# DixianZhu/deBWT

Hardware: NVIDIA B200
Metric: bwt_build_throughput (higher is better)
Workload: dtype u64

## Files before the change

### debwt_b200/csrc/api.cu

```cuda
#include <algorithm>
#include <cstring>
#include <map>
#include <mutex>
#include <string>
#include <tuple>
#include <vector>

#include "../../include/debwt_b200.h"
#include "../../include/debwt_b200_dev.h"
#include "radix_sort.cuh"
#include "stages.cuh"
#include "special.cuh"
#include "ctx.cuh"
#include "dist_kernels.cuh"

namespace debwt {

static thread_local std::string g_err;
unsigned g_launches = 0;
unsigned long long g_launches_total = 0;
void set_error(const std::string& msg) { g_err = msg; }

#define FAIL(msg)            \
    do {                     \
// ... 293 lines not shown
    }
    mark();

    u64 *d_ka = nullptr, *d_kb = nullptr;
    if (dalloc(pool, &d_ka, nk + 2) || dalloc(pool, &d_kb, nk + 2)) return -1;
    if (k_extract(d_text, n, d_seps, R, d_ka, st)) return -1;
    mark();

    void* d_sortws = nullptr;
    if (pool.alloc(&d_sortws, sort_workspace_bytes(nk, c->sort_cfg))) return -1;
    SortWorkspace ws;
    sort_workspace_bind(ws, d_sortws, nk, c->sort_cfg);
    int sweeps = 0;
    ws.ev_sweep_begin = c->ev[11]; ws.ev_sweep_end = c->ev[12]; ws.sweeps_out = &sweeps;
    const unsigned launches_before_sort = g_launches;
    u64* d_keys = nullptr;
    KeyIndex ki;
    ki.bits = key_index_bits(nk);
    if (dalloc(pool, &ki.idx, (1ull << ki.bits) + 2) || k_key_index_init(ki, st)) return -1;
    bool index_marked = false;
    ws.key_index = ki.idx; ws.key_index_bits = ki.bits; ws.key_index_done = &index_marked;
    const bool text_hist = text_digit_hist_applies(n, R);
    if (text_hist && (radix_sort_clear(ws, st) || k_text_digit_hist(d_text, n, d_seps, R, ws.hist, st))) return -1;
    if (radix_sort_u64(d_ka, d_kb, nk, ws, st, &d_keys, text_hist)) return -1;
    S.sort_launches = g_launches - launches_before_sort;
    S.sort_sweeps = (u32)sweeps;
    pool.adopt(d_keys == d_ka ? d_kb : d_ka, (nk + 2) * 8);
    pool.adopt(d_sortws, sort_workspace_bytes(nk, c->sort_cfg));
    u32 h_err[2] = {0, 0};
    CUDA_TRY(cudaMemcpyAsync(h_err, d_err, 8, cudaMemcpyDeviceToHost, st));
    mark();

    u16* d_gmask = nullptr;
    if (dalloc(pool, &d_gmask, nk + 2)) return -1;
    CUDA_TRY(cudaMemsetAsync(d_gmask, 0, (nk + 2) * 2, st));
    if (k_key_index_finish(d_keys, nk, ki, index_marked, st)) return -1;
    if (k_mark_edges(d_keys, nk, ki, d_gmask, st)) return -1;
    if (k_mark_heads_tails(d_text, d_seps, R, d_keys, nk, ki, d_gmask, st)) return -1;
    void* d_brws = nullptr; u64* d_tot = nullptr;
    if (pool.alloc(&d_brws, branch_workspace_bytes(nk)) || dalloc(pool, &d_tot, 4)) return -1;
    if (k_branch_count(d_keys, nk, d_gmask, true, d_brws, d_tot, st)) return -1;
    u64 h_tot[2] = {0, 0};
    CUDA_TRY(cudaMemcpyAsync(h_tot, d_tot, 16, cudaMemcpyDeviceToHost, st));
    CUDA_TRY(cudaStreamSynchronize(st));
    if (h_err[0]) FAIL(c->resolve_ambiguous ? "input contains a symbol that is neither a base nor an IUPAC ambiguity code"
                                            : "input contains a symbol other than A, C, G, T (either case)");
    if (h_err[1] != R) FAIL("input contains '#' or '$' inside a record (they are reserved for the record separators)");
    BranchTable bt;
    bt.n_branch = h_tot[0]; bt.n_blue = h_tot[1];
    S.n_branch = bt.n_branch; S.n_blue = bt.n_blue;
    {
        int bits = 8;
        while (bits < 27 && (1ull << bits) < 2 * bt.n_branch) ++bits;
        bt.bits = bits;
    }
    if (dalloc(pool, &bt.kmer, bt.n_branch + 1) || dalloc(pool, &bt.head, bt.n_branch + 1) ||
        dalloc(pool, &bt.blue, bt.n_branch + 2) || dalloc(pool, &bt.cursor, bt.n_branch + 1) ||
        dalloc(pool, &bt.bidx, BranchTable::index_words(bt.bits)))
        return -1;
    CUDA_TRY(cudaMemsetAsync(bt.cursor, 0, (bt.n_branch + 1) * 4, st));
    if (k_branch_write(d_keys, nk, d_gmask, d_brws, bt, st)) return -1;
    {
        const u32 m32 = (u32)bt.n_blue;
        CUDA_TRY(cudaMemcpyAsync(bt.blue + bt.n_branch, &m32, 4, cudaMemcpyHostToDevice, st));
    }
    if (k_branch_index(bt, st)) return -1;
    int id_bits = 1;
    while (id_bits < 64 && (bt.n_branch >> id_bits)) ++id_bits;
    const bool group_by_sort = id_bits <= 28 && n < (1ull << 32) && bt.n_blue > 1 &&
                               c->blue_grouping == 2;
    bt.hbits = BranchTable::hash_bits(bt.n_branch);
    bt.hmode = group_by_sort ? 0 : 1;
    if (dalloc(pool, &bt.hslots, 1ull << bt.hbits) || k_branch_hash(bt, st)) return -1;
    mark();
// ... 409 lines not shown
    CUDA_TRY(cudaStreamSynchronize(s.st));
    float ms = 0;
    CUDA_TRY(cudaEventElapsedTime(&ms, e0, e1));
    if (ms_out) *ms_out = ms;
    cudaEventDestroy(e0); cudaEventDestroy(e1);
    return 0;
}

int debwt_k_rle(int device, const uint64_t* sorted, uint64_t n, uint64_t* kmers_out, uint64_t* counts_out,
                uint64_t* n_distinct_out) {
    Scratch s;
    if (open_scratch(s, device)) return -1;
    u64 *d_k, *d_km, *d_ct, *d_tot; void* d_ws;
    if (s.get(&d_k, n + 2) || s.get(&d_km, n + 2) || s.get(&d_ct, n + 2) || s.get(&d_tot, 2)) return -1;
    CUDA_TRY(cudaMalloc(&d_ws, rle_workspace_bytes(n)));
    s.ptrs.push_back(d_ws);
    CUDA_TRY(cudaMemcpyAsync(d_k, sorted, n * 8, cudaMemcpyHostToDevice, s.st));
    if (k_rle(d_k, n, d_km, d_ct, d_ws, d_tot, s.st)) return -1;
    u64 d = 0;
    CUDA_TRY(cudaMemcpyAsync(&d, d_tot, 8, cudaMemcpyDeviceToHost, s.st));
    CUDA_TRY(cudaStreamSynchronize(s.st));
    CUDA_TRY(cudaMemcpyAsync(kmers_out, d_km, d * 8, cudaMemcpyDeviceToHost, s.st));
    CUDA_TRY(cudaMemcpyAsync(counts_out, d_ct, d * 8, cudaMemcpyDeviceToHost, s.st));
    CUDA_TRY(cudaStreamSynchronize(s.st));
    if (n_distinct_out) *n_distinct_out = d;
    return 0;
}

int debwt_k_group_masks(int device, const char* text, uint64_t n, const uint64_t* seps, uint64_t R, uint16_t* masks_out) {
    if (check_seps(seps, R, n)) return -1;
    Scratch s;
    if (open_scratch(s, device)) return -1;
    const u64 nk = n - 32 * R;
    u8* d_a; u64 *d_w, *d_s, *d_ka, *d_kb; u32* d_e; u16* d_g; void* d_ws;
    KeyIndex ki;
    ki.bits = key_index_bits(nk);
    if (s.get(&d_a, n + 64) || s.get(&d_w, text_words(n)) || s.get(&d_e, 4) || s.get(&d_s, R) || s.get(&d_ka, nk + 2) ||
        s.get(&d_kb, nk + 2) || s.get(&d_g, nk + 2) || s.get(&ki.idx, (1ull << ki.bits) + 2))
        return -1;
    CUDA_TRY(cudaMalloc(&d_ws, sort_workspace_bytes(nk, 0)));
    s.ptrs.push_back(d_ws);
    SortWorkspace ws;
    sort_workspace_bind(ws, d_ws, nk, 0);
    CUDA_TRY(cudaMemcpyAsync(d_a, text, n, cudaMemcpyHostToDevice, s.st));
    CUDA_TRY(cudaMemcpyAsync(d_s, seps, R * 8, cudaMemcpyHostToDevice, s.st));
    CUDA_TRY(cudaMemsetAsync(d_e, 0, 16, s.st));
    CUDA_TRY(cudaMemsetAsync(d_g, 0, (nk + 2) * 2, s.st));
    u64* d_keys = nullptr;
    if (k_pack(d_a, n, d_w, d_e, s.st) || k_extract(d_w, n, d_s, R, d_ka, s.st) ||
        radix_sort_u64(d_ka, d_kb, nk, ws, s.st, &d_keys) || k_build_key_index(d_keys, nk, ki, s.st) ||
        k_mark_edges(d_keys, nk, ki, d_g, s.st) || k_mark_heads_tails(d_w, d_s, R, d_keys, nk, ki, d_g, s.st) ||
        k_propagate(d_keys, nk, d_g, s.st))
        return -1;
    CUDA_TRY(cudaMemcpyAsync(masks_out, d_g, nk * 2, cudaMemcpyDeviceToHost, s.st));
    CUDA_TRY(cudaStreamSynchronize(s.st));
    return 0;
}


int debwt_k_codes(int device, const char* text, uint64_t n, const uint64_t* seps, uint64_t R, uint8_t* codes_out, uint64_t codes_cap,
                  uint64_t* n_codes_out, uint64_t* blue_head_out, uint64_t* blue_spindex_out, uint8_t* blue_prev_out, uint64_t blue_cap,
                  uint64_t* n_blue_out) {
    debwt_ctx* c = nullptr;
    if (debwt_create(&c, device)) return -1;
    c->cap.on = true;
    int rc = debwt_set_text(c, text, n, seps, R);
    if (!rc) rc = debwt_build(c, 32);
    if (!rc) {
        const auto& q = c->cap;
        if (n_codes_out) *n_codes_out = q.n_codes;
        if (n_blue_out) *n_blue_out = q.blue.size();
        if (q.n_codes > codes_cap || q.blue.size() > blue_cap) { set_error("debwt_k_codes: output buffers too small"); rc = -1; }
    }
    if (!rc) {
        const auto& q = c->cap;
        for (u64 i = 0; i < q.n_codes; ++i) {
            u8 code = (u8)((q.codes[i >> 5] >> (2 * (31 - (i & 31)))) & 3ull);
            if ((q.sep[i >> 5] >> (i & 31)) & 1u) code = i == q.dollar_index ? 5 : 4;
            codes_out[i] = code;
        }
        for (u64 b = 0; b < q.seg_kmer.size(); ++b)
            for (u32 e = q.seg_off[b]; e < q.seg_off[b + 1]; ++e) {
                blue_head_out[e] = q.seg_head[b];
                blue_spindex_out[e] = q.blue[e] >> 4;
                blue_prev_out[e] = (u8)(q.blue[e] & 15ull);
// ... 105 lines not shown
```

### debwt_b200/csrc/stages.cu

```cuda
#include "stages.cuh"

#include <cstdlib>
#include "special.cuh"
#include "stages_dev.cuh"
#include "dist_kernels.cuh"

namespace debwt {

namespace {

constexpr int TPB = 256;
inline unsigned grid_for(u64 work, int per_block) { return (unsigned)((work + per_block - 1) / per_block); }

constexpr int SCAN_ITEMS = 16;
constexpr int SCAN_TILE = TPB * SCAN_ITEMS;

template <bool POPC>
__device__ __forceinline__ u32 scan_f(u32 v) { return POPC ? (u32)__popc(v) : v; }

template <bool POPC>
__global__ void __launch_bounds__(TPB) scan_reduce_kernel(const u32* __restrict__ in, u64 m, u32* __restrict__ part) {
    __shared__ u32 sm[40];
    const u64 base = (u64)blockIdx.x * SCAN_TILE;
    u32 s = 0;
// ... 348 lines not shown
    void* scan_ws = p;
    p += (scan_workspace_bytes(nt) + 7) & ~(size_t)7;
    u64* starts = reinterpret_cast<u64*>(p);
    rle_count_kernel<<<(unsigned)nt, TPB, 0, st>>>(sorted, n, tile_cnt);
    if (scan_exclusive_u32(tile_cnt, tile_ex, nt, false, scan_ws, d_total, st)) return -1;
    rle_write_kernel<<<(unsigned)nt, TPB, 0, st>>>(sorted, n, tile_ex, kmers, starts);
    u64 d = 0;
    CUDA_TRY(cudaMemcpyAsync(&d, d_total, 8, cudaMemcpyDeviceToHost, st));
    CUDA_TRY(cudaStreamSynchronize(st));
    diff_kernel<<<grid_for(d, TPB), TPB, 0, st>>>(starts, d, n, counts);
    DEBWT_COUNT(3);
    CUDA_TRY(cudaGetLastError());
    return 0;
}

namespace {

__global__ void __launch_bounds__(TPB) key_index_mark_kernel(const u64* __restrict__ k, u64 n, KeyIndex ki) {
    const u64 i = (u64)blockIdx.x * TPB + threadIdx.x;
    if (i >= n) return;
    const int sh = 64 - ki.bits;
    const u64 cur = k[i] >> sh;
    if (i == 0 || (k[i - 1] >> sh) != cur) ki.idx[cur] = (u32)i;
}

__global__ void __launch_bounds__(TPB) key_index_fill_kernel(const u64* __restrict__ k, u64 n, KeyIndex ki) {
    const u64 t = (u64)blockIdx.x * TPB + threadIdx.x;
    const u64 nb = 1ull << ki.bits;
    if (t > nb) return;
    if (t == nb) { ki.idx[t] = (u32)n; return; }
    if (ki.idx[t] == 0xFFFFFFFFu) ki.idx[t] = (u32)lower_bound_u64(k, 0, n, t << (64 - ki.bits));
}

constexpr int ME_ROWS = 4;

__device__ __forceinline__ void edge_rows(const u64* __restrict__ k, u64 n, const KeyIndex& ki, u16* __restrict__ gmask, u64 base,
                                          u64 limit) {
    u64 key[ME_ROWS], lo[ME_ROWS], hi[ME_ROWS];
    bool act[ME_ROWS];
#pragma unroll
    for (int j = 0; j < ME_ROWS; ++j) {
        const u64 i = base + (u64)j * TPB;
        act[j] = i < limit;
        key[j] = act[j] ? k[i] : 0;
        if (act[j] && i > 0 && k[i - 1] == key[j]) act[j] = false;
    }
#pragma unroll
    for (int j = 0; j < ME_ROWS; ++j) {
        const u64 t = (key[j] << 2) >> (64 - ki.bits);
        lo[j] = act[j] ? ki.idx[t] : 0;
        hi[j] = act[j] ? ki.idx[t + 1] : 0;
    }
#pragma unroll
    for (int j = 0; j < ME_ROWS; ++j) {
        if (!act[j]) continue;
        const u64 q = key[j] << 2;
        const u64 hs = lower_bound_u64(k, lo[j], hi[j], q);
        if (hs < n && (k[hs] >> 2) == (q >> 2)) atomic_or_u16(gmask, hs, 1u << (u32)(key[j] >> 62));
    }
#pragma unroll
    for (int j = 0; j < ME_ROWS; ++j) {
        if (!act[j]) continue;
        const u64 i = base + (u64)j * TPB;
        atomic_or_u16(gmask, group_head(k, i), 1u << (GM_OUT_SHIFT + (u32)(key[j] & 3)));
    }
}

constexpr u64 ME_TILE = 8192;
constexpr u64 ME_CAP = 8 * ME_TILE;
struct EdgeRun { u64 begin, end; };

__global__ void __launch_bounds__(TPB) edge_bounds_kernel(const u64* __restrict__ k, u64 n, KeyIndex ki, u64 tiles,
                                                         u64* __restrict__ bounds) {
    const u64 x = (u64)blockIdx.x * TPB + threadIdx.x;
    if (x >= 4 * (tiles + 1)) return;
    const u32 c = (u32)(x / (tiles + 1));
    const u64 t = x % (tiles + 1);
    const u64 cbeg = ki.idx[(u64)c << (ki.bits - 2)];
    const u64 cend = (c == 3) ? n : (u64)ki.idx[(u64)(c + 1) << (ki.bits - 2)];
    const u64 a = t * ME_TILE;
    u64 r;
    if (a == 0) r = cbeg;
    else if (a >= n) r = cend;
    else {
        const u64 low = (k[a - 1] >> 2) + 1;
        r = (low >> 62) ? cend : indexed_lower_bound(k, ki, ((u64)c << 62) | low);
    }
    bounds[x] = r;
}

__global__ void __launch_bounds__(TPB) mark_edges_kernel(const u64* __restrict__ k, u64 n, KeyIndex ki, u16* __restrict__ gmask,
                                                        const u64* __restrict__ bounds, u64 tiles, EdgeRun* __restrict__ over,
                                                        u32* __restrict__ n_over) {
    const u32 c = blockIdx.x & 3u;
    const u64 tile = blockIdx.x >> 2;
    const u64 sb = bounds[c * (tiles + 1) + tile];
    u64 se = bounds[c * (tiles + 1) + tile + 1];
    if (se - sb > ME_CAP && se > sb) {
        if (threadIdx.x == 0) over[atomicAdd(n_over, 1u)] = EdgeRun{sb + ME_CAP, se};
        se = sb + ME_CAP;
    }
    for (u64 i0 = sb; i0 < se; i0 += (u64)TPB * ME_ROWS) edge_rows(k, n, ki, gmask, i0 + threadIdx.x, se);
}

__global__ void __launch_bounds__(TPB) mark_edges_over_kernel(const u64* __restrict__ k, u64 n, KeyIndex ki, u16* __restrict__ gmask,
                                                             const EdgeRun* __restrict__ over, const u32* __restrict__ n_over) {
    const u32 m = *n_over;
    for (u32 q = 0; q < m; ++q) {
        const EdgeRun r = over[q];
        for (u64 i0 = r.begin + (u64)blockIdx.x * (TPB * ME_ROWS); i0 < r.end; i0 += (u64)gridDim.x * (TPB * ME_ROWS))
            edge_rows(k, n, ki, gmask, i0 + threadIdx.x, r.end);
    }
}

__global__ void __launch_bounds__(TPB) mark_heads_tails_kernel(const u64* __restrict__ words, const u64* __restrict__ seps,
                                                              u64 n_rec, const u64* __restrict__ k, u64 n, KeyIndex ki,
                                                              u16* __restrict__ gmask) {
    const u64 r = (u64)blockIdx.x * TPB + threadIdx.x;
    if (r >= n_rec) return;
    const u64 start = r ? seps[r - 1] + 1 : 0;
    u64 x = text_window32(words, start) & ~3ull;
    u64 h = indexed_lower_bound(k, ki, x);
    if (h < n && (k[h] & ~3ull) == x) atomic_or_u16(gmask, h, GM_IN_SEP);
    x = text_window32(words, seps[r] - KNODE) & ~3ull;
    h = indexed_lower_bound(k, ki, x);
    if (h < n && (k[h] & ~3ull) == x) atomic_or_u16(gmask, h, GM_OUT_TAIL);
}

__global__ void __launch_bounds__(TPB) propagate_kernel(const u64* __restrict__ k, u64 n, u16* __restrict__ gmask) {
    const u64 i = (u64)blockIdx.x * TPB + threadIdx.x;
    if (i >= n || i == 0) return;
    if ((k[i - 1] >> 2) != (k[i] >> 2)) return;
    gmask[i] = gmask[group_head(k, i)];
}

constexpr int BR_ITEMS = 8;
constexpr int BR_TILE = TPB * BR_ITEMS;

template <bool WRITE, bool PROPAGATE>
__global__ void __launch_bounds__(TPB) branch_kernel(const u64* __restrict__ k, u64 n, u16* __restrict__ gmask,
                                                    u32* __restrict__ tile_nb, u32* __restrict__ tile_blue,
                                                    const u32* __restrict__ tile_nb_ex, const u32* __restrict__ tile_blue_ex,
                                                    u32* __restrict__ head_bits, BranchTable bt) {
    constexpr int NW = TPB / 32;
    __shared__ u32 s_cnt[BR_ITEMS * NW + 1], s_blue[BR_ITEMS * NW + 1];
    if (WRITE && tile_nb[blockIdx.x] == 0) return;
    const int lane = threadIdx.x & 31, warp = threadIdx.x >> 5;
    const u64 base = (u64)blockIdx.x * BR_TILE;
    const u32 lt = lanemask_lt();
    u32 flags[BR_ITEMS], size[BR_ITEMS], bal[BR_ITEMS];
#pragma unroll
    for (int j = 0; j < BR_ITEMS; ++j) {
        const u64 i = base + (u64)j * TPB + threadIdx.x;
        flags[j] = 0;
        size[j] = 0;
        if (WRITE) {
            bal[j] = head_bits[(base + (u64)j * TPB) / 32 + warp];
            if ((bal[j] >> lane) & 1u) {
                const u32 m = gmask[i];
// ... 47 lines not shown
            if (lane >= o) { ic += tc; ib += tb; }
        }
        const u32 ec = ic - (c0 + c1), eb = ib - (b0 + b1);
        s_cnt[2 * lane] = ec; s_cnt[2 * lane + 1] = ec + c0;
        s_blue[2 * lane] = eb; s_blue[2 * lane + 1] = eb + b0;
        if (lane == 31) {
            s_cnt[BR_ITEMS * NW] = ic; s_blue[BR_ITEMS * NW] = ib;
            if (!WRITE) { tile_nb[blockIdx.x] = ic; tile_blue[blockIdx.x] = ib; }
        }
    }
    if (!WRITE) return;
    __syncthreads();
    const u64 ob0 = tile_nb_ex[blockIdx.x];
    const u32 ol0 = tile_blue_ex[blockIdx.x];
#pragma unroll
    for (int j = 0; j < BR_ITEMS; ++j) {
        if (bal[j] == 0) continue;
        u32 inc = size[j];
#pragma unroll
        for (int o = 1; o < 32; o <<= 1) {
            const u32 t = __shfl_up_sync(0xffffffffu, inc, o);
            if (lane >= o) inc += t;
        }
        if (flags[j]) {
            const u64 i = base + (u64)j * TPB + threadIdx.x;
            const u64 ob = ob0 + s_cnt[j * NW + warp] + __popc(bal[j] & lt);
            bt.kmer[ob] = (k[i] & ~3ull) | (flags[j] & 3u);
            bt.head[ob] = (u32)i;
            bt.blue[ob] = ol0 + s_blue[j * NW + warp] + (inc - size[j]);
        }
    }
}

__global__ void __launch_bounds__(TPB) branch_index_kernel(BranchTable bt) {
    const u64 t = (u64)blockIdx.x * TPB + threadIdx.x;
    const u64 nb = 1ull << bt.bits;
    if (t > nb) return;
    bt.bidx[t] = (t == nb) ? (u32)bt.n_branch : (u32)lower_bound_u64(bt.kmer, 0, bt.n_branch, t << (64 - bt.bits));
}

__global__ void __launch_bounds__(TPB) branch_filter_kernel(BranchTable bt) {
    const u64 b = (u64)blockIdx.x * TPB + threadIdx.x;
    if (b >= bt.n_branch) return;
    const u64 f = bt.filter_of(bt.kmer[b] & ~3ull);
    atomicOr(bt.filter() + (f >> 5), 1u << (f & 31));
}

__global__ void __launch_bounds__(TPB) branch_hash_kernel(BranchTable bt) {
    const u64 b = (u64)blockIdx.x * TPB + threadIdx.x;
    if (b >= bt.n_branch) return;
    const u64 e = bt.kmer[b];
    const u64 mask = (1ull << bt.hbits) - 1;
    for (u64 h = bt.hash_of(e & ~3ull);; h = (h + 1) & mask) {
        unsigned long long* claim = reinterpret_cast<unsigned long long*>(&bt.hslots[h].x);
        if (atomicCAS(claim, 0ull, (unsigned long long)e) == 0ull) {
            bt.hslots[h].y = bt.hmode ? (u64)bt.blue[b] << 32 : b;
            return;
        }
    }
}

__global__ void __launch_bounds__(TPB) special_ins_kernel(const u64* __restrict__ k, u64 n, KeyIndex ki,
                                                         const u64* __restrict__ pads, u64 m, u64* __restrict__ ins) {
    const u64 t = (u64)blockIdx.x * TPB + threadIdx.x;
    if (t < m) ins[t] = indexed_upper_bound(k, ki, pads[t]);
}

}

int k_key_index_init(KeyIndex ki, cudaStream_t st) {
    CUDA_TRY(cudaMemsetAsync(ki.idx, 0xFF, ((1ull << ki.bits) + 1) * 4, st));
    return 0;
}

int k_key_index_finish(const u64* sorted, u64 n, KeyIndex ki, bool marked, cudaStream_t st) {
    if (n && !marked) {
        key_index_mark_kernel<<<grid_for(n, TPB), TPB, 0, st>>>(sorted, n, ki);
        DEBWT_COUNT(1);
    }
    key_index_fill_kernel<<<grid_for((1ull << ki.bits) + 1, TPB), TPB, 0, st>>>(sorted, n, ki);
    DEBWT_COUNT(1);
    CUDA_TRY(cudaGetLastError());
    return 0;
}

int k_build_key_index(const u64* sorted, u64 n, KeyIndex ki, cudaStream_t st) {
    if (k_key_index_init(ki, st)) return -1;
    return k_key_index_finish(sorted, n, ki, false, st);
}

int k_mark_edges(const u64* sorted, u64 n, KeyIndex ki, u16* gmask, cudaStream_t st) {
    if (n == 0) return 0;
    const u64 tiles = (n + ME_TILE - 1) / ME_TILE;
    const u64 cap = n / ME_CAP + 8;
    char* ws = nullptr;
    CUDA_TRY(cudaMallocAsync(reinterpret_cast<void**>(&ws), 16 + cap * sizeof(EdgeRun) + 4 * (tiles + 1) * 8, st));
    u32* n_over = reinterpret_cast<u32*>(ws);
    EdgeRun* over = reinterpret_cast<EdgeRun*>(ws + 16);
    u64* bounds = reinterpret_cast<u64*>(ws + 16 + cap * sizeof(EdgeRun));
    cudaMemsetAsync(n_over, 0, 16, st);
    edge_bounds_kernel<<<grid_for(4 * (tiles + 1), TPB), TPB, 0, st>>>(sorted, n, ki, tiles, bounds);
    mark_edges_kernel<<<(unsigned)(4 * tiles), TPB, 0, st>>>(sorted, n, ki, gmask, bounds, tiles, over, n_over);
    mark_edges_over_kernel<<<148 * 8, TPB, 0, st>>>(sorted, n, ki, gmask, over, n_over);
    DEBWT_COUNT(3);
    const cudaError_t e = cudaGetLastError();
    cudaFreeAsync(ws, st);
    if (e != cudaSuccess) { set_error(std::string("mark_edges: ") + cudaGetErrorString(e)); return -1; }
    return 0;
}

int k_mark_heads_tails(const u64* words, const u64* d_seps, u64 n_rec, const u64* sorted, u64 n, KeyIndex ki, u16* gmask,
                       cudaStream_t st) {
    mark_heads_tails_kernel<<<grid_for(n_rec, TPB), TPB, 0, st>>>(words, d_seps, n_rec, sorted, n, ki, gmask);
    DEBWT_COUNT(1);
    CUDA_TRY(cudaGetLastError());
    return 0;
}

int k_propagate(const u64* sorted, u64 n, u16* gmask, cudaStream_t st) {
    if (n == 0) return 0;
    propagate_kernel<<<grid_for(n, TPB), TPB, 0, st>>>(sorted, n, gmask);
    DEBWT_COUNT(1);
    CUDA_TRY(cudaGetLastError());
    return 0;
}

namespace {
struct BranchWs { u32 *nb, *blue, *nb_ex, *blue_ex, *head_bits; void* scan_ws; u64 nt; };
BranchWs branch_ws(void* workspace, u64 n) {
    BranchWs w;
    w.nt = (n + BR_TILE - 1) / BR_TILE;
    u32* p = reinterpret_cast<u32*>(workspace);
    w.nb = p; w.blue = p + w.nt; w.nb_ex = p + 2 * w.nt; w.blue_ex = p + 3 * w.nt;
    char* q = reinterpret_cast<char*>(p + 4 * w.nt);
    q += (8 - (reinterpret_cast<uintptr_t>(q) & 7)) & 7;
    w.scan_ws = q;
    q += (scan_workspace_bytes(w.nt + 1) + 15) & ~(size_t)15;
    w.head_bits = reinterpret_cast<u32*>(q);
    return w;
}
}

size_t branch_workspace_bytes(u64 n) {
    const u64 nt = (n + BR_TILE - 1) / BR_TILE + 1;
    return nt * 16 + 16 + scan_workspace_bytes(nt) + 32 + nt * (BR_TILE / 8);
}

int k_branch_count(const u64* sorted, u64 n, u16* gmask, bool propagate, void* workspace, u64* d_totals, cudaStream_t st) {
    BranchWs w = branch_ws(workspace, n);
    BranchTable none;
    if (propagate) branch_kernel<false, true><<<(unsigned)w.nt, TPB, 0, st>>>(sorted, n, gmask, w.nb, w.blue, nullptr, nullptr, w.head_bits, none);
    else branch_kernel<false, false><<<(unsigned)w.nt, TPB, 0, st>>>(sorted, n, gmask, w.nb, w.blue, nullptr, nullptr, w.head_bits, none);
    DEBWT_COUNT(1);
    if (scan_exclusive_u32(w.nb, w.nb_ex, w.nt, false, w.scan_ws, d_totals, st)) return -1;
    if (scan_exclusive_u32(w.blue, w.blue_ex, w.nt, false, w.scan_ws, d_totals + 1, st)) return -1;
    CUDA_TRY(cudaGetLastError());
    return 0;
}

int k_branch_write(const u64* sorted, u64 n, const u16* gmask, void* workspace, BranchTable bt, cudaStream_t st) {
    BranchWs w = branch_ws(workspace, n);
    branch_kernel<true, false><<<(unsigned)w.nt, TPB, 0, st>>>(sorted, n, const_cast<u16*>(gmask), w.nb, nullptr, w.nb_ex, w.blue_ex, w.head_bits, bt);
    DEBWT_COUNT(1);
    CUDA_TRY(cudaGetLastError());
    return 0;
}

int k_branch_index(BranchTable bt, cudaStream_t st) {
    branch_index_kernel<<<grid_for((1ull << bt.bits) + 1, TPB), TPB, 0, st>>>(bt);
    CUDA_TRY(cudaMemsetAsync(bt.filter(), 0, (1ull << (BranchTable::filter_bits(bt.bits) - 5)) * 4, st));
    if (bt.n_branch) branch_filter_kernel<<<grid_for(bt.n_branch, TPB), TPB, 0, st>>>(bt);
    DEBWT_COUNT(2);
    CUDA_TRY(cudaGetLastError());
    return 0;
}

int k_branch_hash(BranchTable bt, cudaStream_t st) {
    if (!bt.hslots) return 0;
    CUDA_TRY(cudaMemsetAsync(bt.hslots, 0, (1ull << bt.hbits) * sizeof(ulonglong2), st));
    if (bt.n_branch) branch_hash_kernel<<<grid_for(bt.n_branch, TPB), TPB, 0, st>>>(bt);
    DEBWT_COUNT(1);
    CUDA_TRY(cudaGetLastError());
    return 0;
}

namespace {
__global__ void __launch_bounds__(128) special_scan_kernel(const u64* __restrict__ words, const u64* __restrict__ seps,
                                                          u64 n_rec, const u64* __restrict__ k, u64 n_keys, KeyIndex ki,
                                                          SpecialInfo* __restrict__ out) {
// ... 628 lines not shown
```

### debwt_b200/csrc/stages.cuh

```cuda
#pragma once
#include "common.cuh"

namespace debwt {

size_t scan_workspace_bytes(u64 m);
int scan_exclusive_u32(const u32* in, u32* out, u64 m, bool popc, void* workspace, u64* d_total, cudaStream_t st);

struct PackPolicy {
    bool resolve = false;
    u64 seed = 0;
    u64 pos_base = 0;
};
int k_pack(const u8* ascii, u64 n, u64* words, u32* d_err, cudaStream_t st, PackPolicy pol = PackPolicy());
inline u64 text_words(u64 n) { return (n + 32 + 31) / 32 + 1; }
int k_extract(const u64* words, u64 n, const u64* d_seps, u64 n_rec, u64* keys, cudaStream_t st);
int k_extract_slice(const u64* words, u64 n, u64 pos_lo, u64 pos_hi, const u64* d_seps, u64 n_rec, u64 idx_base, u64* keys,
                    cudaStream_t st);

bool text_digit_hist_applies(u64 n, u64 n_rec);
int k_text_digit_hist(const u64* words, u64 n, const u64* d_seps, u64 n_rec, u64* ghist, cudaStream_t st);

int k_rle(const u64* sorted, u64 n, u64* kmers, u64* counts, void* workspace, u64* d_total, cudaStream_t st);
size_t rle_workspace_bytes(u64 n);

struct KeyIndex {
    u32* idx = nullptr;
    int bits = 0;
};
inline int key_index_bits(u64 n) {
    int b = 8;
    while (b < 28 && (8ull << b) < n) ++b;
    return b;
}
int k_build_key_index(const u64* sorted, u64 n, KeyIndex ki, cudaStream_t st);
int k_key_index_init(KeyIndex ki, cudaStream_t st);
int k_key_index_finish(const u64* sorted, u64 n, KeyIndex ki, bool marked, cudaStream_t st);
__host__ __device__ __forceinline__ u64 indexed_lower_bound(const u64* __restrict__ k, const KeyIndex& ki, u64 q) {
    const u64 t = q >> (64 - ki.bits);
    return lower_bound_u64(k, ki.idx[t], ki.idx[t + 1], q);
}
__host__ __device__ __forceinline__ u64 indexed_upper_bound(const u64* __restrict__ k, const KeyIndex& ki, u64 q) {
    const u64 t = q >> (64 - ki.bits);
    return upper_bound_u64(k, ki.idx[t], ki.idx[t + 1], q);
}

int k_mark_edges(const u64* sorted, u64 n, KeyIndex ki, u16* gmask, cudaStream_t st);
int k_mark_heads_tails(const u64* words, const u64* d_seps, u64 n_rec, const u64* sorted, u64 n, KeyIndex ki, u16* gmask,
                       cudaStream_t st);
int k_propagate(const u64* sorted, u64 n, u16* gmask, cudaStream_t st);

struct BranchTable {
    u64 n_branch = 0;
    u64 n_blue = 0;
    u64* kmer = nullptr;
    u32* head = nullptr;
    u32* blue = nullptr;
    u32* cursor = nullptr;
    u32* bidx = nullptr;
    int bits = 0;
    ulonglong2* hslots = nullptr;
    int hbits = 0;
    int hmode = 0;
    __host__ __device__ static int hash_bits(u64 n_branch) { int b = 10; while (b < 40 && (1ull << b) < 3 * n_branch) ++b; return b; }
    __host__ __device__ u64 hash_of(u64 x) const { return ((x >> 2) * 0x9E3779B97F4A7C15ull) >> (64 - hbits); }
    __host__ __device__ u64 filter_of(u64 x) const { return ((x >> 2) * 0x9E3779B97F4A7C15ull) >> (64 - filter_bits(bits)); }
    __host__ __device__ static int filter_bits(int bits) { return bits + 3 < 30 ? bits + 3 : 30; }
    __host__ __device__ static u64 index_words(int bits) { return (1ull << bits) + 2 + (1ull << (filter_bits(bits) - 5)); }
    __host__ __device__ u32* filter() const { return bidx + (1ull << bits) + 2; }
};
size_t branch_workspace_bytes(u64 n);
int k_branch_count(const u64* sorted, u64 n, u16* gmask, bool propagate, void* workspace, u64* d_totals, cudaStream_t st);
int k_branch_write(const u64* sorted, u64 n, const u16* gmask, void* workspace, BranchTable bt, cudaStream_t st);
int k_branch_index(BranchTable bt, cudaStream_t st);
int k_branch_hash(BranchTable bt, cudaStream_t st);

int k_special_insertion(const u64* sorted, u64 n, KeyIndex ki, const u64* pads, u64 m, u64* ins, cudaStream_t st);

int k_flag_positions(const u64* words, u64 n, const u64* d_seps, u64 n_rec, BranchTable bt, u32* mo_bits, u64* blue,
                     cudaStream_t st);
int k_flag_positions_keys(const u64* words, u64 n, const u64* d_seps, u64 n_rec, BranchTable bt, int shift, u32* mo_bits,
                          u64* bkeys, u64* d_counter, cudaStream_t st);
int k_blue_keys_fix(u64* bkeys, u64 m, const u32* mo_bits, const u32* word_prefix, cudaStream_t st);
int k_blue_keys_strip(u64* bkeys, u64 m, cudaStream_t st);
int k_blue_fix_interleaved(u64* blue, u64 m, const u32* mo_bits, const u32* word_prefix, u64 n_words, u64* scratch, cudaStream_t st);
int k_patch_bits(u32* mo_bits, const u64* positions, u64 m, cudaStream_t st);
int k_emit_codes(const u64* words, u64 n, const u32* mo_bits, const u32* word_prefix, u64* sp_codes, cudaStream_t st);
int k_mark_sep_codes(const u32* mo_bits, const u32* word_prefix, const u64* positions, u64 m, u32* sp_sep,
                     u64* d_code_index_out, cudaStream_t st);
int k_blue_fix(u64* blue, u64 m, const u32* mo_bits, const u32* word_prefix, cudaStream_t st);

struct SpView {
    const u64* codes;
    const u32* sep;
    u64 dollar_index;
    u64 n_codes;
    const u32* sep_sum = nullptr;
};
int k_sort_blue(u64* blue, BranchTable bt, SpView sp, u32* d_work , cudaStream_t st);

int k_fill_case2(const u16* gmask, u64 n_keys, u64 n, const u64* spec_rows, u64 m, u64* bwt, cudaStream_t st);
int k_emit_blue(const u64* blue, BranchTable bt, const u64* spec_ins, u64 m, u64* bwt, u64* sharp_rows,
                u32* d_sharp_count, u64* dollar_row, cudaStream_t st);
int k_emit_special(const u64* spec_rows, const u8* spec_chr, u64 m, u64* bwt, cudaStream_t st);

// ... 2 lines not shown
```

Before: 9020.

## Fuse edge marking, head/tail marking, propagation and branch count into one tiled classify kernel

```diff
diff --git a/debwt_b200/csrc/api.cu b/debwt_b200/csrc/api.cu
--- a/debwt_b200/csrc/api.cu
+++ b/debwt_b200/csrc/api.cu
@@ -349,14 +349,10 @@
     mark();
 
     u16* d_gmask = nullptr;
-    if (dalloc(pool, &d_gmask, nk + 2)) return -1;
-    CUDA_TRY(cudaMemsetAsync(d_gmask, 0, (nk + 2) * 2, st));
+    void* d_brws = nullptr; u64* d_tot = nullptr;
+    if (dalloc(pool, &d_gmask, nk + 2) || pool.alloc(&d_brws, branch_workspace_bytes(nk)) || dalloc(pool, &d_tot, 4)) return -1;
     if (k_key_index_finish(d_keys, nk, ki, index_marked, st)) return -1;
-    if (k_mark_edges(d_keys, nk, ki, d_gmask, st)) return -1;
-    if (k_mark_heads_tails(d_text, d_seps, R, d_keys, nk, ki, d_gmask, st)) return -1;
-    void* d_brws = nullptr; u64* d_tot = nullptr;
-    if (pool.alloc(&d_brws, branch_workspace_bytes(nk)) || dalloc(pool, &d_tot, 4)) return -1;
-    if (k_branch_count(d_keys, nk, d_gmask, true, d_brws, d_tot, st)) return -1;
+    if (k_classify(d_text, d_seps, R, d_keys, nk, ki, d_gmask, d_brws, d_tot, st)) return -1;
     u64 h_tot[2] = {0, 0};
     CUDA_TRY(cudaMemcpyAsync(h_tot, d_tot, 16, cudaMemcpyDeviceToHost, st));
     CUDA_TRY(cudaStreamSynchronize(st));
@@ -832,11 +828,12 @@
     Scratch s;
     if (open_scratch(s, device)) return -1;
     const u64 nk = n - 32 * R;
-    u8* d_a; u64 *d_w, *d_s, *d_ka, *d_kb; u32* d_e; u16* d_g; void* d_ws;
+    u8* d_a; u64 *d_w, *d_s, *d_ka, *d_kb, *d_tot; u32* d_e; u16* d_g; void* d_ws; u8* d_brws;
     KeyIndex ki;
     ki.bits = key_index_bits(nk);
     if (s.get(&d_a, n + 64) || s.get(&d_w, text_words(n)) || s.get(&d_e, 4) || s.get(&d_s, R) || s.get(&d_ka, nk + 2) ||
-        s.get(&d_kb, nk + 2) || s.get(&d_g, nk + 2) || s.get(&ki.idx, (1ull << ki.bits) + 2))
+        s.get(&d_kb, nk + 2) || s.get(&d_g, nk + 2) || s.get(&ki.idx, (1ull << ki.bits) + 2) ||
+        s.get(&d_brws, branch_workspace_bytes(nk)) || s.get(&d_tot, 2))
         return -1;
     CUDA_TRY(cudaMalloc(&d_ws, sort_workspace_bytes(nk, 0)));
     s.ptrs.push_back(d_ws);
@@ -845,12 +842,10 @@
     CUDA_TRY(cudaMemcpyAsync(d_a, text, n, cudaMemcpyHostToDevice, s.st));
     CUDA_TRY(cudaMemcpyAsync(d_s, seps, R * 8, cudaMemcpyHostToDevice, s.st));
     CUDA_TRY(cudaMemsetAsync(d_e, 0, 16, s.st));
-    CUDA_TRY(cudaMemsetAsync(d_g, 0, (nk + 2) * 2, s.st));
     u64* d_keys = nullptr;
     if (k_pack(d_a, n, d_w, d_e, s.st) || k_extract(d_w, n, d_s, R, d_ka, s.st) ||
         radix_sort_u64(d_ka, d_kb, nk, ws, s.st, &d_keys) || k_build_key_index(d_keys, nk, ki, s.st) ||
-        k_mark_edges(d_keys, nk, ki, d_g, s.st) || k_mark_heads_tails(d_w, d_s, R, d_keys, nk, ki, d_g, s.st) ||
-        k_propagate(d_keys, nk, d_g, s.st))
+        k_classify(d_w, d_s, R, d_keys, nk, ki, d_g, d_brws, d_tot, s.st))
         return -1;
     CUDA_TRY(cudaMemcpyAsync(masks_out, d_g, nk * 2, cudaMemcpyDeviceToHost, s.st));
     CUDA_TRY(cudaStreamSynchronize(s.st));
diff --git a/debwt_b200/csrc/stages.cu b/debwt_b200/csrc/stages.cu
--- a/debwt_b200/csrc/stages.cu
+++ b/debwt_b200/csrc/stages.cu
@@ -404,43 +404,10 @@
     if (ki.idx[t] == 0xFFFFFFFFu) ki.idx[t] = (u32)lower_bound_u64(k, 0, n, t << (64 - ki.bits));
 }
 
-constexpr int ME_ROWS = 4;
-
-__device__ __forceinline__ void edge_rows(const u64* __restrict__ k, u64 n, const KeyIndex& ki, u16* __restrict__ gmask, u64 base,
-                                          u64 limit) {
-    u64 key[ME_ROWS], lo[ME_ROWS], hi[ME_ROWS];
-    bool act[ME_ROWS];
-#pragma unroll
-    for (int j = 0; j < ME_ROWS; ++j) {
-        const u64 i = base + (u64)j * TPB;
-        act[j] = i < limit;
-        key[j] = act[j] ? k[i] : 0;
-        if (act[j] && i > 0 && k[i - 1] == key[j]) act[j] = false;
-    }
-#pragma unroll
-    for (int j = 0; j < ME_ROWS; ++j) {
-        const u64 t = (key[j] << 2) >> (64 - ki.bits);
-        lo[j] = act[j] ? ki.idx[t] : 0;
-        hi[j] = act[j] ? ki.idx[t + 1] : 0;
-    }
-#pragma unroll
-    for (int j = 0; j < ME_ROWS; ++j) {
-        if (!act[j]) continue;
-        const u64 q = key[j] << 2;
-        const u64 hs = lower_bound_u64(k, lo[j], hi[j], q);
-        if (hs < n && (k[hs] >> 2) == (q >> 2)) atomic_or_u16(gmask, hs, 1u << (u32)(key[j] >> 62));
-    }
-#pragma unroll
-    for (int j = 0; j < ME_ROWS; ++j) {
-        if (!act[j]) continue;
-        const u64 i = base + (u64)j * TPB;
-        atomic_or_u16(gmask, group_head(k, i), 1u << (GM_OUT_SHIFT + (u32)(key[j] & 3)));
-    }
-}
-
-constexpr u64 ME_TILE = 8192;
-constexpr u64 ME_CAP = 8 * ME_TILE;
-struct EdgeRun { u64 begin, end; };
+constexpr int CT_TPB = 256;
+constexpr int CT_TILE = 32 * CT_TPB;
+constexpr int CT_SRC = 8;
+constexpr u64 CT_CAP = 8 * CT_TILE;
 
 __global__ void __launch_bounds__(TPB) edge_bounds_kernel(const u64* __restrict__ k, u64 n, KeyIndex ki, u64 tiles,
                                                          u64* __restrict__ bounds) {
@@ -450,7 +417,7 @@
     const u64 t = x % (tiles + 1);
     const u64 cbeg = ki.idx[(u64)c << (ki.bits - 2)];
     const u64 cend = (c == 3) ? n : (u64)ki.idx[(u64)(c + 1) << (ki.bits - 2)];
-    const u64 a = t * ME_TILE;
+    const u64 a = t * CT_TILE;
     u64 r;
     if (a == 0) r = cbeg;
     else if (a >= n) r = cend;
@@ -461,42 +428,25 @@
     bounds[x] = r;
 }
 
-__global__ void __launch_bounds__(TPB) mark_edges_kernel(const u64* __restrict__ k, u64 n, KeyIndex ki, u16* __restrict__ gmask,
-                                                        const u64* __restrict__ bounds, u64 tiles, EdgeRun* __restrict__ over,
-                                                        u32* __restrict__ n_over) {
-    const u32 c = blockIdx.x & 3u;
-    const u64 tile = blockIdx.x >> 2;
-    const u64 sb = bounds[c * (tiles + 1) + tile];
-    u64 se = bounds[c * (tiles + 1) + tile + 1];
-    if (se - sb > ME_CAP && se > sb) {
-        if (threadIdx.x == 0) over[atomicAdd(n_over, 1u)] = EdgeRun{sb + ME_CAP, se};
-        se = sb + ME_CAP;
-    }
-    for (u64 i0 = sb; i0 < se; i0 += (u64)TPB * ME_ROWS) edge_rows(k, n, ki, gmask, i0 + threadIdx.x, se);
-}
-
-__global__ void __launch_bounds__(TPB) mark_edges_over_kernel(const u64* __restrict__ k, u64 n, KeyIndex ki, u16* __restrict__ gmask,
-                                                             const EdgeRun* __restrict__ over, const u32* __restrict__ n_over) {
-    const u32 m = *n_over;
-    for (u32 q = 0; q < m; ++q) {
-        const EdgeRun r = over[q];
-        for (u64 i0 = r.begin + (u64)blockIdx.x * (TPB * ME_ROWS); i0 < r.end; i0 += (u64)gridDim.x * (TPB * ME_ROWS))
-            edge_rows(k, n, ki, gmask, i0 + threadIdx.x, r.end);
-    }
-}
-
+template <bool BITMAP>
 __global__ void __launch_bounds__(TPB) mark_heads_tails_kernel(const u64* __restrict__ words, const u64* __restrict__ seps,
                                                               u64 n_rec, const u64* __restrict__ k, u64 n, KeyIndex ki,
-                                                              u16* __restrict__ gmask) {
+                                                              u16* __restrict__ gmask, u32* __restrict__ sent) {
     const u64 r = (u64)blockIdx.x * TPB + threadIdx.x;
     if (r >= n_rec) return;
     const u64 start = r ? seps[r - 1] + 1 : 0;
     u64 x = text_window32(words, start) & ~3ull;
     u64 h = indexed_lower_bound(k, ki, x);
-    if (h < n && (k[h] & ~3ull) == x) atomic_or_u16(gmask, h, GM_IN_SEP);
+    if (h < n && (k[h] & ~3ull) == x) {
+        if (BITMAP) atomicOr(sent + (h >> 4), 1u << (2 * (h & 15)));
+        else atomic_or_u16(gmask, h, GM_IN_SEP);
+    }
     x = text_window32(words, seps[r] - KNODE) & ~3ull;
     h = indexed_lower_bound(k, ki, x);
-    if (h < n && (k[h] & ~3ull) == x) atomic_or_u16(gmask, h, GM_OUT_TAIL);
+    if (h < n && (k[h] & ~3ull) == x) {
+        if (BITMAP) atomicOr(sent + (h >> 4), 2u << (2 * (h & 15)));
+        else atomic_or_u16(gmask, h, GM_OUT_TAIL);
+    }
 }
 
 __global__ void __launch_bounds__(TPB) propagate_kernel(const u64* __restrict__ k, u64 n, u16* __restrict__ gmask) {
@@ -610,6 +560,263 @@
     }
 }
 
+static_assert(CT_TILE % BR_TILE == 0, "a classify tile covers whole branch tiles");
+constexpr int CT_SEGS = CT_TILE / 32;
+constexpr int CT_BR = CT_TILE / BR_TILE;
+
+struct OverRun { u64 begin, end; u32 mask; };
+
+struct ClassifyShared {
+    u64 key[CT_TILE + 2];
+    u32 mask[CT_TILE / 2];
+    u32 hb[CT_SEGS];
+    int prev[CT_SEGS];
+    int next[CT_SEGS];
+    int wmax[CT_TPB / 32], wmin[CT_TPB / 32];
+    u32 sent[CT_TILE / 16];
+    u32 cnt[CT_BR], blue[CT_BR];
+    int last_head;
+    u64 last_end;
+};
+
+__device__ __forceinline__ void smask_or(ClassifyShared& S, int h, u32 bits) {
+    atomicOr(&S.mask[h >> 1], bits << (16 * (h & 1)));
+}
+__device__ __forceinline__ u32 smask_get(const ClassifyShared& S, int h) { return (S.mask[h >> 1] >> (16 * (h & 1))) & 0xFFFFu; }
+
+__device__ __forceinline__ int gallop_lower_bound(const u64* s, int p, int m, u64 q) {
+    if (p >= m || s[p] >= q) return p;
+    int lo = p, step = 1;
+    while (lo + step < m && s[lo + step] < q) { lo += step; step <<= 1; }
+    int hi = lo + step < m ? lo + step : m;
+    ++lo;
+    while (lo < hi) {
+        const int mid = (lo + hi) >> 1;
+        if (s[mid] < q) lo = mid + 1; else hi = mid;
+    }
+    return lo;
+}
+
+__device__ __forceinline__ int head_of(const ClassifyShared& S, int i, u32 hb) {
+    const u32 le = hb & (0xFFFFFFFFu >> (31 - (i & 31)));
+    return le ? (i & ~31) + 31 - __clz(le) : S.prev[i >> 5];
+}
+
+__global__ void __launch_bounds__(CT_TPB, 2) classify_tile_kernel(const u64* __restrict__ k, u64 n, KeyIndex ki, const u64* __restrict__ bounds,
+                                                                 u64 tiles, const u32* __restrict__ sent, u64 sent_words,
+                                                                 u16* __restrict__ gmask,
+                                                                 u32* __restrict__ tile_nb, u32* __restrict__ tile_blue,
+                                                                 u32* __restrict__ head_bits, u64 br_tiles,
+                                                                 OverRun* __restrict__ over, u32* __restrict__ n_over) {
+    extern __shared__ __align__(16) unsigned char ct_smem[];
+    ClassifyShared& S = *reinterpret_cast<ClassifyShared*>(ct_smem);
+    const int tid = threadIdx.x, lane = tid & 31, warp = tid >> 5;
+    const u64 a = (u64)blockIdx.x * CT_TILE;
+    const int m = n - a < (u64)CT_TILE ? (int)(n - a) : CT_TILE;
+
+#pragma unroll
+    for (int j = 0; j < CT_TILE / 2 / CT_TPB; ++j) {
+        const int v = j * CT_TPB + tid;
+        if (2 * v + 1 < m) {
+            const u32 dst = (u32)__cvta_generic_to_shared(&S.key[2 + 2 * v]);
+            asm volatile("cp.async.cg.shared.global [%0], [%1], 16;" ::"r"(dst), "l"(k + a + 2 * v) : "memory");
+        } else {
+            S.key[2 + 2 * v] = 2 * v < m ? k[a + 2 * v] : 0;
+            S.key[3 + 2 * v] = 0;
+        }
+    }
+    asm volatile("cp.async.commit_group;" ::: "memory");
+    u64 run_pos[4], run_end_[4];
+#pragma unroll
+    for (int c = 0; c < 4; ++c) {
+        run_pos[c] = bounds[c * (tiles + 1) + blockIdx.x];
+        run_end_[c] = bounds[c * (tiles + 1) + blockIdx.x + 1];
+    }
+    constexpr int CH = CT_TPB * CT_SRC;
+    u64 src[4][CT_SRC];
+#pragma unroll
+    for (int c = 0; c < 4; ++c) {
+        const u64 p0 = run_pos[c] + (u64)tid * CT_SRC;
+#pragma unroll
+        for (int e = 0; e < CT_SRC; ++e) src[c][e] = p0 + e < run_end_[c] ? k[p0 + e] : 0;
+    }
+    for (int i = tid; i < CT_TILE / 2; i += CT_TPB) S.mask[i] = 0;
+    for (int i = tid; i < CT_TILE / 16; i += CT_TPB) S.sent[i] = a / 16 + i < sent_words ? sent[a / 16 + i] : 0;
+    if (tid < CT_BR) { S.cnt[tid] = 0; S.blue[tid] = 0; }
+    if (tid == 0) S.key[1] = a ? k[a - 1] : 0;
+    if (tid == 1) S.key[0] = a + m < n ? k[a + m] : 0;
+    asm volatile("cp.async.wait_all;" ::: "memory");
+    __syncthreads();
+
+#pragma unroll 4
+    for (int j = 0; j < CT_SEGS / (CT_TPB / 32); ++j) {
+        const int i = j * CT_TPB + tid;
+        const bool head = i < m && (a + i == 0 || (S.key[2 + i] >> 2) != (S.key[1 + i] >> 2));
+        const u32 hb = __ballot_sync(0xFFFFFFFFu, head);
+        if (lane == 0) S.hb[i >> 5] = hb;
+    }
+    __syncthreads();
+
+    {
+        const u32 hb = S.hb[tid];
+        int mx = hb ? tid * 32 + 31 - __clz(hb) : -1;
+        int mn = hb ? tid * 32 + __ffs(hb) - 1 : CT_TILE;
+#pragma unroll
+        for (int o = 1; o < 32; o <<= 1) {
+            const int u = __shfl_up_sync(0xFFFFFFFFu, mx, o), d = __shfl_down_sync(0xFFFFFFFFu, mn, o);
+            if (lane >= o) mx = max(mx, u);
+            if (lane + o < 32) mn = min(mn, d);
+        }
+        if (lane == 31) S.wmax[warp] = mx;
+        if (lane == 0) S.wmin[warp] = mn;
+        __syncthreads();
+        int cmax = -1, cmin = CT_TILE;
+        for (int w = 0; w < warp; ++w) cmax = max(cmax, S.wmax[w]);
+        for (int w = warp + 1; w < CT_TPB / 32; ++w) cmin = min(cmin, S.wmin[w]);
+        const int up = __shfl_up_sync(0xFFFFFFFFu, mx, 1), down = __shfl_down_sync(0xFFFFFFFFu, mn, 1);
+        S.prev[tid] = max(cmax, lane ? up : -1);
+        S.next[tid] = min(cmin, lane < 31 ? down : CT_TILE);
+        if (tid == CT_TPB - 1) {
+            const int h = max(cmax, mx);
+            S.last_head = (h >= 0 && m == CT_TILE && a + m < n && (S.key[0] >> 2) == (S.key[1 + m] >> 2)) ? h : -1;
+        }
+    }
+    __syncthreads();
+
+#pragma unroll 4
+    for (int j = 0; j < CT_SEGS / (CT_TPB / 32); ++j) {
+        const int i = j * CT_TPB + tid;
+        if (i >= m) break;
+        const u64 key = S.key[2 + i];
+        const int h = head_of(S, i, S.hb[i >> 5]);
+        if (h < 0) continue;
+        u32 bits = (a + i == 0 || key != S.key[1 + i]) ? 1u << (GM_OUT_SHIFT + (u32)(key & 3)) : 0u;
+        if (h == i) {
+            const u32 sm = (S.sent[i >> 4] >> (2 * (i & 15))) & 3u;
+            bits |= (sm & 1u ? GM_IN_SEP : 0u) | (sm & 2u ? GM_OUT_TAIL : 0u);
+        }
+        if (bits) smask_or(S, h, bits);
+    }
+
+    if (tid >= CT_TPB - 5 && S.last_head >= 0) {
+        const u64 x = S.key[0] >> 2;
+        const u32 b = CT_TPB - 1 - tid;
+        if (b < 4) {
+            const u64 q = (x << 2) | b;
+            const u64 p = indexed_lower_bound(k, ki, q);
+            if (p < n && k[p] == q) smask_or(S, S.last_head, 1u << (GM_OUT_SHIFT + b));
+        } else {
+            S.last_end = x == (1ull << 62) - 1 ? n : indexed_lower_bound(k, ki, (x + 1) << 2);
+        }
+    }
+
+    const u64* tk = S.key + 2;
+#pragma unroll
+    for (u32 c = 0; c < 4; ++c) {
+        const u64 cnt0 = run_end_[c] - run_pos[c] < (u64)CH ? run_end_[c] - run_pos[c] : (u64)CH;
+        int p = 0;
+        u64 prev = ~0ull;
+#pragma unroll
+        for (int e = 0; e < CT_SRC; ++e) {
+            if ((u64)tid * CT_SRC + e >= cnt0) break;
+            const u64 q = src[c][e] << 2;
+            if (q == prev) continue;
+            prev = q;
+            p = e ? gallop_lower_bound(tk, p, m, q) : (int)lower_bound_u64(tk, 0, m, q);
+            if (p < m && (tk[p] & ~3ull) == q) smask_or(S, p, 1u << c);
+        }
+        const u64 se = run_end_[c];
+        u64 pos = run_pos[c] + cnt0;
+        while (pos < se) {
+            const u64 cnt = se - pos < (u64)CH ? se - pos : (u64)CH;
+            const u64 p0 = pos + (u64)tid * CT_SRC;
+            u64 v[CT_SRC];
+#pragma unroll
+            for (int e = 0; e < CT_SRC; ++e) v[e] = p0 + e < pos + cnt ? k[p0 + e] : 0;
+            const u64 first = k[pos], lastk = k[pos + cnt - 1];
+            if (cnt == (u64)CH && first == lastk) {
+                if (tid == 0) {
+                    const u64 q = first << 2;
+                    const int h = (int)lower_bound_u64(tk, 0, m, q);
+                    if (h < m && (tk[h] & ~3ull) == q) smask_or(S, h, 1u << c);
+                }
+                const u64 probe = pos + (u64)(tid + 2) * CH - 1;
+                const int more = __syncthreads_count(probe < se && k[probe] == first);
+                pos += (u64)(more + 1) * CH;
+                continue;
+            }
+            p = 0;
+            prev = ~0ull;
+#pragma unroll
+            for (int e = 0; e < CT_SRC; ++e) {
+                if (p0 + e >= pos + cnt) break;
+                const u64 q = v[e] << 2;
+                if (q == prev) continue;
+                prev = q;
+                p = e ? gallop_lower_bound(tk, p, m, q) : (int)lower_bound_u64(tk, 0, m, q);
+                if (p < m && (tk[p] & ~3ull) == q) smask_or(S, p, 1u << c);
+            }
+            pos += cnt;
+        }
+    }
+    __syncthreads();
+
+    const u64 end_last = S.last_head >= 0 ? S.last_end : a + m;
+    const u64 hb_words = br_tiles * (BR_TILE / 32);
+#pragma unroll 2
+    for (int j = 0; j < CT_SEGS / (CT_TPB / 32); ++j) {
+        const int i = j * CT_TPB + tid;
+        const u32 hb = S.hb[i >> 5];
+        u32 f = 0, size = 0;
+        if (i < m) {
+            const int h = head_of(S, i, hb);
+            if (h >= 0) {
+                const u32 mk = smask_get(S, h);
+                gmask[a + i] = (u16)mk;
+                if (h == i) {
+                    f = (gm_multi_out(mk) ? 1u : 0u) | (gm_multi_in(mk) ? 2u : 0u);
+                    if (f & 2u) {
+                        const u32 above = hb & ~(0xFFFFFFFFu >> (31 - lane));
+                        const int nx = above ? (i & ~31) + __ffs(above) - 1 : S.next[i >> 5];
+                        size = nx < CT_TILE ? (u32)(nx - i) : (u32)(end_last - (a + i));
+                    }
+                }
+            }
+        }
+        const u32 bal = __ballot_sync(0xFFFFFFFFu, f != 0);
+        const u64 w = (a >> 5) + (u64)(i >> 5);
+        if (lane == 0 && w < hb_words) head_bits[w] = bal;
+        if (bal) {
+#pragma unroll
+            for (int o = 16; o; o >>= 1) size += __shfl_xor_sync(0xFFFFFFFFu, size, o);
+            if (lane == 0) {
+                atomicAdd(&S.cnt[(j * CT_TPB) / BR_TILE], (u32)__popc(bal));
+                atomicAdd(&S.blue[(j * CT_TPB) / BR_TILE], size);
+            }
+        }
+    }
+    if (S.last_head >= 0) {
+        const u16 mk = (u16)smask_get(S, S.last_head);
+        const u64 b = a + m, e = S.last_end, stop = e - b > CT_CAP ? b + CT_CAP : e;
+        for (u64 i = b + tid; i < stop; i += CT_TPB) gmask[i] = mk;
+        if (tid == 0 && stop < e) over[atomicAdd(n_over, 1u)] = OverRun{stop, e, mk};
+    }
+    __syncthreads();
+    if (tid < CT_BR && (u64)blockIdx.x * CT_BR + tid < br_tiles) {
+        tile_nb[(u64)blockIdx.x * CT_BR + tid] = S.cnt[tid];
+        tile_blue[(u64)blockIdx.x * CT_BR + tid] = S.blue[tid];
+    }
+}
+
+__global__ void __launch_bounds__(TPB) classify_over_kernel(u16* __restrict__ gmask, const OverRun* __restrict__ over,
+                                                           const u32* __restrict__ n_over) {
+    const u32 m = *n_over;
+    for (u32 q = 0; q < m; ++q) {
+        const OverRun r = over[q];
+        for (u64 i = r.begin + (u64)blockIdx.x * TPB + threadIdx.x; i < r.end; i += (u64)gridDim.x * TPB) gmask[i] = (u16)r.mask;
+    }
+}
+
 __global__ void __launch_bounds__(TPB) branch_index_kernel(BranchTable bt) {
     const u64 t = (u64)blockIdx.x * TPB + threadIdx.x;
     const u64 nb = 1ull << bt.bits;
@@ -667,29 +874,9 @@
     return k_key_index_finish(sorted, n, ki, false, st);
 }
 
-int k_mark_edges(const u64* sorted, u64 n, KeyIndex ki, u16* gmask, cudaStream_t st) {
-    if (n == 0) return 0;
-    const u64 tiles = (n + ME_TILE - 1) / ME_TILE;
-    const u64 cap = n / ME_CAP + 8;
-    char* ws = nullptr;
-    CUDA_TRY(cudaMallocAsync(reinterpret_cast<void**>(&ws), 16 + cap * sizeof(EdgeRun) + 4 * (tiles + 1) * 8, st));
-    u32* n_over = reinterpret_cast<u32*>(ws);
-    EdgeRun* over = reinterpret_cast<EdgeRun*>(ws + 16);
-    u64* bounds = reinterpret_cast<u64*>(ws + 16 + cap * sizeof(EdgeRun));
-    cudaMemsetAsync(n_over, 0, 16, st);
-    edge_bounds_kernel<<<grid_for(4 * (tiles + 1), TPB), TPB, 0, st>>>(sorted, n, ki, tiles, bounds);
-    mark_edges_kernel<<<(unsigned)(4 * tiles), TPB, 0, st>>>(sorted, n, ki, gmask, bounds, tiles, over, n_over);
-    mark_edges_over_kernel<<<148 * 8, TPB, 0, st>>>(sorted, n, ki, gmask, over, n_over);
-    DEBWT_COUNT(3);
-    const cudaError_t e = cudaGetLastError();
-    cudaFreeAsync(ws, st);
-    if (e != cudaSuccess) { set_error(std::string("mark_edges: ") + cudaGetErrorString(e)); return -1; }
-    return 0;
-}
-
 int k_mark_heads_tails(const u64* words, const u64* d_seps, u64 n_rec, const u64* sorted, u64 n, KeyIndex ki, u16* gmask,
                        cudaStream_t st) {
-    mark_heads_tails_kernel<<<grid_for(n_rec, TPB), TPB, 0, st>>>(words, d_seps, n_rec, sorted, n, ki, gmask);
+    mark_heads_tails_kernel<false><<<grid_for(n_rec, TPB), TPB, 0, st>>>(words, d_seps, n_rec, sorted, n, ki, gmask, nullptr);
     DEBWT_COUNT(1);
     CUDA_TRY(cudaGetLastError());
     return 0;
@@ -717,6 +904,10 @@
     w.head_bits = reinterpret_cast<u32*>(q);
     return w;
 }
+int branch_scans(const BranchWs& w, u64* d_totals, cudaStream_t st) {
+    if (scan_exclusive_u32(w.nb, w.nb_ex, w.nt, false, w.scan_ws, d_totals, st)) return -1;
+    return scan_exclusive_u32(w.blue, w.blue_ex, w.nt, false, w.scan_ws, d_totals + 1, st);
+}
 }
 
 size_t branch_workspace_bytes(u64 n) {
@@ -730,9 +921,40 @@
     if (propagate) branch_kernel<false, true><<<(unsigned)w.nt, TPB, 0, st>>>(sorted, n, gmask, w.nb, w.blue, nullptr, nullptr, w.head_bits, none);
     else branch_kernel<false, false><<<(unsigned)w.nt, TPB, 0, st>>>(sorted, n, gmask, w.nb, w.blue, nullptr, nullptr, w.head_bits, none);
     DEBWT_COUNT(1);
-    if (scan_exclusive_u32(w.nb, w.nb_ex, w.nt, false, w.scan_ws, d_totals, st)) return -1;
-    if (scan_exclusive_u32(w.blue, w.blue_ex, w.nt, false, w.scan_ws, d_totals + 1, st)) return -1;
-    CUDA_TRY(cudaGetLastError());
+    if (branch_scans(w, d_totals, st)) return -1;
+    CUDA_TRY(cudaGetLastError());
+    return 0;
+}
+
+int k_classify(const u64* words, const u64* d_seps, u64 n_rec, const u64* sorted, u64 n, KeyIndex ki, u16* gmask, void* workspace,
+               u64* d_totals, cudaStream_t st) {
+    if (n == 0) { CUDA_TRY(cudaMemsetAsync(d_totals, 0, 16, st)); return 0; }
+    BranchWs w = branch_ws(workspace, n);
+    const u64 tiles = (n + CT_TILE - 1) / CT_TILE;
+    const u64 cap = n / CT_CAP + 8;
+    const u64 sent_words = n / 16 + 1;
+    const size_t over_bytes = (cap * sizeof(OverRun) + 15) & ~(size_t)15;
+    char* ws = nullptr;
+    CUDA_TRY(cudaMallocAsync(reinterpret_cast<void**>(&ws), 16 + over_bytes + 4 * (tiles + 1) * 8 + sent_words * 4, st));
+    u32* n_over = reinterpret_cast<u32*>(ws);
+    OverRun* over = reinterpret_cast<OverRun*>(ws + 16);
+    u64* bounds = reinterpret_cast<u64*>(ws + 16 + over_bytes);
+    u32* sent = reinterpret_cast<u32*>(bounds + 4 * (tiles + 1));
+    cudaMemsetAsync(n_over, 0, 16, st);
+    cudaMemsetAsync(sent, 0, sent_words * 4, st);
+    mark_heads_tails_kernel<true><<<grid_for(n_rec, TPB), TPB, 0, st>>>(words, d_seps, n_rec, sorted, n, ki, nullptr, sent);
+    edge_bounds_kernel<<<grid_for(4 * (tiles + 1), TPB), TPB, 0, st>>>(sorted, n, ki, tiles, bounds);
+    cudaFuncSetAttribute(classify_tile_kernel, cudaFuncAttributeMaxDynamicSharedMemorySize, (int)sizeof(ClassifyShared));
+    cudaFuncSetAttribute(classify_tile_kernel, cudaFuncAttributePreferredSharedMemoryCarveout, cudaSharedmemCarveoutMaxShared);
+    classify_tile_kernel<<<(unsigned)tiles, CT_TPB, sizeof(ClassifyShared), st>>>(sorted, n, ki, bounds, tiles, sent, sent_words, gmask,
+                                                                               w.nb, w.blue,
+                                                                               w.head_bits, w.nt, over, n_over);
+    classify_over_kernel<<<148 * 8, TPB, 0, st>>>(gmask, over, n_over);
+    DEBWT_COUNT(4);
+    cudaError_t e = cudaGetLastError();
+    if (e == cudaSuccess && branch_scans(w, d_totals, st)) e = cudaErrorUnknown;
+    cudaFreeAsync(ws, st);
+    if (e != cudaSuccess) { set_error(std::string("classify: ") + cudaGetErrorString(e)); return -1; }
     return 0;
 }
 
diff --git a/debwt_b200/csrc/stages.cuh b/debwt_b200/csrc/stages.cuh
--- a/debwt_b200/csrc/stages.cuh
+++ b/debwt_b200/csrc/stages.cuh
@@ -44,7 +44,6 @@
     return upper_bound_u64(k, ki.idx[t], ki.idx[t + 1], q);
 }
 
-int k_mark_edges(const u64* sorted, u64 n, KeyIndex ki, u16* gmask, cudaStream_t st);
 int k_mark_heads_tails(const u64* words, const u64* d_seps, u64 n_rec, const u64* sorted, u64 n, KeyIndex ki, u16* gmask,
                        cudaStream_t st);
 int k_propagate(const u64* sorted, u64 n, u16* gmask, cudaStream_t st);
@@ -70,6 +69,8 @@
 };
 size_t branch_workspace_bytes(u64 n);
 int k_branch_count(const u64* sorted, u64 n, u16* gmask, bool propagate, void* workspace, u64* d_totals, cudaStream_t st);
+int k_classify(const u64* words, const u64* d_seps, u64 n_rec, const u64* sorted, u64 n, KeyIndex ki, u16* gmask, void* workspace,
+               u64* d_totals, cudaStream_t st);
 int k_branch_write(const u64* sorted, u64 n, const u16* gmask, void* workspace, BranchTable bt, cudaStream_t st);
 int k_branch_index(BranchTable bt, cudaStream_t st);
 int k_branch_hash(BranchTable bt, cudaStream_t st);
```

Measured after the change: 8687, median of 6. 0.963x the previous value.
